# jankammeth/BA-path-planning

Hardware: AMD Instinct MI355X
Metric: SCP iterations/sec (N agents x K waypoints) (higher is better)
Workload: dtype f64

## Files before the change

### ba-path-planning_amd/csrc/scp_qp_persist16.hip

```cpp
#include "scp_qp_persist_device.h"

namespace {
using namespace scpdev;
using namespace scp_persist;

#ifdef SCP_PHASE_PROFILE
__device__ unsigned long long scp_persist16_clk[16];
#define PSTAMP(slot)                                           \
  do {                                                         \
    if (prof_t) {                                              \
      const unsigned long long now_ = wall_clock64();          \
      pacc_s[slot] += now_ - pacc_s[15];                       \
      pacc_s[15] = now_;                                       \
    }                                                          \
  } while (0)
#else
#define PSTAMP(slot) ((void)0)
#endif

constexpr int nct_of(int D, int APB) { return (D * APB + 15) / 16; }
constexpr int AB_STRIDE = 32;

constexpr bool t_on_mfma(int D, int APB) { return 4 * nct_of(D, APB) < APB && APB <= 8; }
constexpr int ent_doubles(int D) { return D + 6; }

struct Lds16 {
  int RSK, tK, nks;
  size_t rt, pt, qt, ml, tl, gp, ab, gchk, ent, n_dbl;
  __host__ __device__ Lds16(int K, int cap, int nblk, int D, int APB) {
    const int NC16 = 16 * nct_of(D, APB), APB16 = APB;
    const bool tq = t_on_mfma(D, APB);
    RSK = pad_col(K);
    tK = (K + 15) >> 4;
    nks = (K + 3) >> 2;
    size_t o = 0;
    rt = o; o += (size_t)NC16 * RSK;
    pt = o; o += (size_t)NC16 * RSK;
    ml = o; o += (size_t)tK * nks * 64;
    qt = pt;
    tl = ml;
    if (tq) {
      qt = o; o += (size_t)NC16 * RSK;
      tl = o; o += (size_t)tK * nks * 64;
    }
    gp = o; o += (size_t)2 * nblk;
    ab = o; o += (size_t)APB16 * AB_STRIDE;
    if ((size_t)2 * NC16 * RSK >= (size_t)NCHK * nblk) gchk = rt;
    else { gchk = o; o += (size_t)NCHK * nblk; }
    ent = o; o += (size_t)cap * ent_doubles(D);
    n_dbl = o;
  }
};

template <int D, int APB16>
__global__ __launch_bounds__(64 * APB16) void cg1_persist16_kernel(PersistArgs A) {
  constexpr int NT16 = 64 * APB16;
  constexpr int NCT = nct_of(D, APB16);
  constexpr int NC16 = 16 * NCT;
  constexpr bool TQ = t_on_mfma(D, APB16);
  extern __shared__ __attribute__((aligned(16))) double lds[];
  __shared__ double red[NCHK][APB16];
  __shared__ double cert_s[3][APB16];
  __shared__ double chk_s[NCHK];
  __shared__ int fail_s;
#ifdef SCP_PHASE_PROFILE
  __shared__ unsigned long long pacc_s[16];
  const bool prof_t = blockIdx.x == gridDim.x / 2 && threadIdx.x == 0;
  if (prof_t) {
    for (int i = 0; i < 15; ++i) pacc_s[i] = 0;
    pacc_s[15] = wall_clock64();
  }
#endif
  const int K = A.K, N = A.N;
  const int64_t C = A.C;
  const int cap = A.ent_cap, nblk = A.nblk;
  const Lds16 L(K, cap, nblk, D, APB16);
  const int RSK = L.RSK, tK = L.tK, nks = L.nks;
  double* Rt = lds + L.rt;
  double* Pt = lds + L.pt;
  double* Qt = lds + L.qt;
  double* Ml = lds + L.ml;
  double* Tl = lds + L.tl;
  double* gp = lds + L.gp;
  double* ab = lds + L.ab;
  double* gck = lds + L.gchk;
  double* e_c = lds + L.ent;
  double* e_l = e_c + (size_t)cap * D;
  double* e_z = e_l + cap;
  double* e_y = e_z + cap;
  double* e_g = e_y + cap;
  double* e_ax = e_g + cap;
  double* e_s = e_ax + cap;
  int* e_code = (int*)(lds + L.n_dbl);
  int* cptr = e_code + cap;

  const int wave = threadIdx.x >> 6, lane = threadIdx.x & 63;
  const int a0 = blockIdx.x * APB16;
  const int agent = a0 + wave;
  const bool aok = agent < N;
  const int k = lane;
  const bool live = aok && k < K;
  const bool jok = live && k < K - 1;
  const bool lastk = k == K - 1;
  const double h = A.h, hh = h * h, ih = 1.0 / h, alpha = A.alpha;
  double rho = A.rho, rho_c = A.rho_c;
  unsigned n_rho = 0;

  const int a1 = min(a0 + APB16, N);
  const int ebase = A.cell_ptr[cell_of(0, a0, K)];
  const int ne = A.cell_ptr[cell_of(0, a1, K)] - ebase;
  if (entries_overflow<APB16>(A)) return;
  if (threadIdx.x == 0) fail_s = 0;
  for (int i = threadIdx.x; i <= (a1 - a0) * K; i += NT16) cptr[i] = A.cell_ptr[cell_of(0, a0, K) + i] - ebase;
  for (int e = threadIdx.x; e < ne; e += NT16) {
    const int code = A.ent_code[ebase + e];
    const int n = code >> 1, side = code & 1;
    const int wi = A.w_i[n], wj = A.w_j[n], wk = A.w_k[n];
    const int own = side ? wj : wi, par = side ? wi : wj;
    e_code[e] = wk | ((own - a0) << 6) | (side << 10) | (par << 11);
    const int64_t bo = (int64_t)wk * C + (int64_t)own * D, bp = (int64_t)wk * C + (int64_t)par * D;
    double ax = 0.0;
#pragma unroll
    for (int d = 0; d < D; ++d) {
      const double eta = A.w_eta[(size_t)n * D + d];
      const double c = side ? -eta : eta;
      e_c[(size_t)e * D + d] = c;
      ax += c * (A.Qx[bo + d] - A.Qx[bp + d]);
    }
    e_ax[e] = ax;
    e_l[e] = A.w_l[n];
    e_z[e] = A.zc[n];
    e_y[e] = A.yc[n];
    e_g[e] = A.gval[ebase + e];
  }
  for (int i = threadIdx.x; i < NC16 * RSK; i += NT16) Rt[i] = 0.0;
  for (int i = threadIdx.x; i < tK * nks * 64; i += NT16) {
    Ml[i] = A.pMinv[i];
    if constexpr (TQ) Tl[i] = A.pT[i];
  }

  double v[D][4], off[D], x[D], c1[D], c2[D];
#pragma unroll
  for (int t = 0; t < 4; ++t) {
    const bool rok = t == 0 ? jok : live;
    const int row = t == 0 ? k : t * K - 1 + k;
    const double rr = (t >= 2 && lastk) ? rho * A.rho_eq : rho;
#pragma unroll
    for (int d = 0; d < D; ++d) {
      v[d][t] = 0.0;
      if (rok) {
        const int64_t g = (int64_t)row * C + (int64_t)agent * D + d;
        v[d][t] = A.zf[g] + A.yf[g] / rr;
      }
    }
  }
  if (threadIdx.x < APB16 * D) {
    const int al = threadIdx.x / D, d = threadIdx.x % D, ag = a0 + al;
    double* o = ab + al * AB_STRIDE;
    const bool there = ag < N;
    const double v0 = there ? A.states[((size_t)N + ag) * D + d] : 0.0;
    o[d] = A.vel_lo - v0;
    o[4 + d] = A.vel_hi - v0;
    o[8 + d] = (there ? A.states[((size_t)3 * N + ag) * D + d] : 0.0) - v0;
    o[12 + d] = A.pmin[d];
    o[16 + d] = A.pmax[d];
    o[20 + d] = there ? A.states[((size_t)2 * N + ag) * D + d] : 0.0;
    o[24 + d] = -1e300;
    o[28 + d] = 1e300;
  }
#pragma unroll
  for (int d = 0; d < D; ++d) {
#pragma clang fp contract(off)
    const double p0 = aok ? A.states[(size_t)agent * D + d] : 0.0, v0 = aok ? A.states[((size_t)N + agent) * D + d] : 0.0;
    const double hk = h * (double)(k + 1);
    const double hkv = hk * v0;
    off[d] = p0 + hkv;
  }
  const double* const tb = ab + wave * AB_STRIDE;
  const double* const b_vl = tb + (live ? (lastk ? 8 : 0) : 24);
  const double* const b_vh = tb + (live ? (lastk ? 8 : 4) : 28);
  const double* const b_pl = tb + (live ? (lastk ? 20 : 12) : 24);
  const double* const b_ph = tb + (live ? (lastk ? 20 : 16) : 28);
  auto bounds = [&](int d, double (&lo)[2], double (&hi)[2]) {
    lo[0] = b_vl[d];
    hi[0] = b_vh[d];
    lo[1] = b_pl[d] - off[d];
    hi[1] = b_ph[d] - off[d];
  };
#pragma unroll
  for (int d = 0; d < D; ++d) {
    x[d] = live ? A.x[(int64_t)k * C + (int64_t)agent * D + d] : 0.0;
    const double s1 = wave_incl_sum(x[d]);
    const double s2 = lane_below(wave_incl_sum(s1));
    c1[d] = live ? s1 : 0.0;
    c2[d] = live ? s2 : 0.0;
  }
  const double jlo = A.jerk_lo, jhi = A.jerk_hi, alo = A.acc_lo, ahi = A.acc_hi;
  __syncthreads();
  const int c0 = aok ? cptr[wave * K + min(k, K - 1)] : 0;
  const int c1e = (aok && k < K) ? cptr[wave * K + k + 1] : c0;
  const bool has_rows = c1e > c0;
  u64* my_cell = A.cells + ((size_t)((int64_t)min(k, K - 1) * N + (aok ? agent : 0)) * D) * 2;
  double* my_pt = Pt + (size_t)(wave * D) * RSK + k;
  double* my_rt = Rt + (size_t)(wave * D) * RSK + k;

  PSTAMP(0);
  bool ok = true;
  int it_done = A.it0;
  unsigned steps = 0;
  unsigned exit_code = 0;
  const bool with_dy = A.eps_prim_inf > 0.0;
  if (threadIdx.x < 3 * APB16) (&cert_s[0][0])[threadIdx.x] = 0.0;
  int cad = A.cad0;
  for (;;) {
  int nit = cad - it_done % cad;
  if (it_done + nit > A.max_iter) nit = A.max_iter - it_done;
  for (int it = 0; it < nit; ++it, ++steps) {
    const unsigned tag = A.epoch0 + steps + 1u;
    const bool last = it == nit - 1;
    const bool first = A.first_step && steps == 0u;
    u64* gpart = A.gpart + (size_t)(tag & 1u) * nblk * 4;
    const double rv = lastk ? rho * A.rho_eq : rho;
    {
      double r[D];
      double g[D];
#pragma unroll
      for (int d = 0; d < D; ++d) g[d] = 0.0;
      for (int e = c0; e < c1e; ++e) {
        const double ge = e_g[e];
#pragma unroll
        for (int d = 0; d < D; ++d) g[d] += e_c[(size_t)e * D + d] * ge;
      }
#pragma unroll
      for (int d = 0; d < D; ++d) {
        double lo[2], hi[2];
        bounds(d, lo, hi);
        const double xn = lane_above(x[d]);
        double cj = fmin(fmax(v[d][0], jlo), jhi), ca = fmin(fmax(v[d][1], alo), ahi);
        double cv = fmin(fmax(v[d][2], lo[0]), hi[0]), cp = fmin(fmax(v[d][3], lo[1]), hi[1]);
        if (first) { cj = v[d][0]; ca = v[d][1]; cv = v[d][2]; cp = v[d][3]; }
        const double wj = jok ? rho * ((cj - (xn - x[d]) * ih) - (v[d][0] - cj)) : 0.0;
        const double wa = rho * ((ca - x[d]) - (v[d][1] - ca));
        const double wv = rv * ((cv - h * c1[d]) - (v[d][2] - cv));
        const double wp = rv * ((cp - hh * (c2[d] + 0.5 * c1[d])) - (v[d][3] - cp));
        const double u1 = h * wv + 0.5 * hh * (wp - g[d]);
        const double u2 = wp + g[d];
        const double d1 = wave_incl_rsum(u1);
        const double s1 = wave_incl_rsum(u2);
        const double d2 = lane_above(wave_incl_rsum(s1));
        const double wjm = lane_below(wj);
        r[d] = (((wjm - wj) * ih + wa) + (d1 + 0.5 * hh * g[d]) + hh * d2) - 2.0 * x[d];
        if (live) my_rt[d * RSK] = r[d];
        __builtin_amdgcn_sched_barrier(0);
      }
    }
    __syncthreads();
    PSTAMP(1);
    if ((wave < 4 * NCT || (TQ && wave < 4 * NCT + 4)) && (wave & 3) < tK) {
      const bool tw = TQ && wave >= 4 * NCT;
      const int li = lane & 15, lk = lane >> 4;
      const int tile = wave & 3, ct = tw ? 0 : wave >> 2;
      const double* Mt = (tw ? Tl : Ml) + (size_t)tile * nks * 64 + lane;
      const double* Bt = Rt + (size_t)(ct * 16 + li) * RSK;
      double4_t acc = {0.0, 0.0, 0.0, 0.0};
#pragma unroll 4
      for (int s = 0; s < nks; ++s) {
        const int kk = 4 * s + lk;
        const double b = kk < K ? Bt[kk] : 0.0;
        acc = __builtin_amdgcn_mfma_f64_16x16x4f64(Mt[(size_t)s * 64], b, acc, 0, 0, 0);
      }
      if (TQ && tw) {
        const int al = li / D, d = li % D;
        const bool col_ok = li < D * APB16 && a0 + al < N;
        double* Ot = Qt + (size_t)li * RSK;
#pragma unroll
        for (int q = 0; q < 4; ++q) {
          const int row = tile * 16 + lk + 4 * q;
          if (row < K) {
            Ot[row] = acc[q];
            if (col_ok && cptr[al * K + row + 1] > cptr[al * K + row])
              st_granules(A.cells + ((size_t)((int64_t)row * N + a0 + al) * D + d) * 2, tag, acc[q]);
          }
        }
      } else {
        double* Ot = Pt + (size_t)(ct * 16 + li) * RSK;
#pragma unroll
        for (int q = 0; q < 4; ++q) {
          const int row = tile * 16 + lk + 4 * q;
          if (row < K) Ot[row] = acc[q];
        }
      }
    }
    __syncthreads();
    PSTAMP(2);
    double p[D], s1p[D], s2p[D];
    {
      double rz = 0.0;
#pragma unroll
      for (int d = 0; d < D; ++d) {
        p[d] = live ? my_pt[d * RSK] : 0.0;
        rz += (live ? my_rt[d * RSK] : 0.0) * p[d];
        const double cs1 = wave_incl_sum(p[d]);
        const double cs2 = lane_below(wave_incl_sum(cs1));
        s1p[d] = live ? cs1 : 0.0;
        s2p[d] = live ? cs2 : 0.0;
        if constexpr (!TQ) {
          const double qp = hh * (cs2 - 0.5 * lane_below(cs1));
          if (has_rows) {
            st_granules(my_cell + 2 * d, tag, qp);
            my_pt[d * RSK] = qp;
          }
        }
      }
      rz = wave_incl_sum(rz);
      if (lane == 63) red[0][wave] = rz;
    }
    if constexpr (!TQ) __syncthreads();
    PSTAMP(3);
    {
      double sq = 0.0;
      unsigned spins = 0;
      bool bad = false;
      for (int e = threadIdx.x; e < ne; e += NT16) {
        const int code = e_code[e];
        const int ek = code & 63, al = (code >> 6) & 15, side = (code >> 10) & 1, par = code >> 11;
        const u64* pc = A.cells + ((size_t)((int64_t)ek * N + par) * D) * 2;
        u32x4 w[D];
        if (!wait_cell<D>(A, pc, tag, spins, w)) {
          bad = true;
          break;
        }
        double s = 0.0;
#pragma unroll
        for (int d = 0; d < D; ++d) s += e_c[(size_t)e * D + d] * (Qt[(size_t)(al * D + d) * RSK + ek] - pair_value(w[d]));
        e_s[e] = s;
        if (!side) sq += s * s;
      }
      if (bad) raise_give_up(A, fail_s);
      sq = wave_incl_sum(sq);
      if (lane == 63) red[1][wave] = sq;
    }
    __syncthreads();
    if (fail_s) { ok = false; break; }
    PSTAMP(4);
    publish_partials(red, 2, 3u, gpart + (size_t)blockIdx.x * 4, tag);
    double zcl[D][4];
#pragma unroll
    for (int d = 0; d < D; ++d) {
      double lo[2], hi[2];
      bounds(d, lo, hi);
      zcl[d][0] = fmin(fmax(v[d][0], jlo), jhi);
      zcl[d][1] = fmin(fmax(v[d][1], alo), ahi);
      zcl[d][2] = fmin(fmax(v[d][2], lo[0]), hi[0]);
      zcl[d][3] = fmin(fmax(v[d][3], lo[1]), hi[1]);
      if (first) {
#pragma unroll
        for (int t = 0; t < 4; ++t) zcl[d][t] = v[d][t];
      }
    }
    gather_pairs<NT16>(A, gpart, 2 * nblk, tag, gp, fail_s);
    __syncthreads();
    if (fail_s) { ok = false; break; }
    PSTAMP(5);
    const double a = step_length(gp, nblk, rho_c);
    const double aa = alpha * a;
    PSTAMP(6);
    {
      const double irc = 1.0 / rho_c;
      for (int e = threadIdx.x; e < ne; e += NT16) {
        const double s = e_s[e], ax0 = e_ax[e];
        const double tc = fma(a, s, ax0), ax = fma(aa, s, ax0);
        e_ax[e] = ax;
        const double zo = e_z[e], yo = e_y[e];
        const double zh = alpha * tc + (1.0 - alpha) * zo;
        const double zn = fmax(zh + yo * irc, e_l[e]);
        const double yn = yo + rho_c * (zh - zn);
        e_z[e] = zn;
        e_y[e] = yn;
        e_g[e] = (rho_c * zn - yn) - rho_c * ax;
        if (last && with_dy) e_s[e] = fmin(yn - yo, 0.0);
      }
    }
    const bool cert = last && with_dy;
    if (cert) __syncthreads();
    double m_ndy = 0.0, m_supp = 0.0, m_natdy = 0.0;
    {
#pragma unroll
      for (int d = 0; d < D; ++d) {
        const double xt = fma(a, p[d], x[d]);
        const double t1 = fma(a, s1p[d], c1[d]), t2 = fma(a, s2p[d], c2[d]);
        const double xtn = lane_above(xt);
        const double cj = zcl[d][0], ca = zcl[d][1], cv = zcl[d][2], cp = zcl[d][3];
        const double nj = jok ? fma(alpha, (xtn - xt) * ih - cj, v[d][0]) : v[d][0];
        const double na = fma(alpha, xt - ca, v[d][1]);
        const double nv = fma(alpha, h * t1 - cv, v[d][2]);
        const double np = fma(alpha, hh * (t2 + 0.5 * t1) - cp, v[d][3]);
        if (cert) {
          double lo[2], hi[2];
          bounds(d, lo, hi);
          const double dyj = rho * ((nj - fmin(fmax(nj, jlo), jhi)) - (v[d][0] - cj));
          const double dya = rho * ((na - fmin(fmax(na, alo), ahi)) - (v[d][1] - ca));
          const double dyv = rv * ((nv - fmin(fmax(nv, lo[0]), hi[0])) - (v[d][2] - cv));
          const double dyp = rv * ((np - fmin(fmax(np, lo[1]), hi[1])) - (v[d][3] - cp));
          m_ndy = fmax(m_ndy, fmax(fmax(fabs(dyj), fabs(dya)), fmax(fabs(dyv), fabs(dyp))));
          m_supp += (jhi * fmax(dyj, 0.0) + jlo * fmin(dyj, 0.0)) + (ahi * fmax(dya, 0.0) + alo * fmin(dya, 0.0)) +
                    (hi[0] * fmax(dyv, 0.0) + lo[0] * fmin(dyv, 0.0)) + (hi[1] * fmax(dyp, 0.0) + lo[1] * fmin(dyp, 0.0));
          double gd = 0.0;
          for (int e = c0; e < c1e; ++e) gd += e_c[(size_t)e * D + d] * e_s[e];
          const double u1 = h * dyv + 0.5 * hh * (dyp - gd);
          const double u2 = dyp + gd;
          const double d1 = wave_incl_rsum(u1);
          const double s1 = wave_incl_rsum(u2);
          const double d2 = lane_above(wave_incl_rsum(s1));
          const double vjm = lane_below(dyj);
          const double at = ((vjm - dyj) * ih + dya) + (d1 + 0.5 * hh * gd) + hh * d2;
          if (live) m_natdy = fmax(m_natdy, fabs(at));
        }
        v[d][0] = nj; v[d][1] = na; v[d][2] = nv; v[d][3] = np;
        x[d] = fma(aa, p[d], x[d]);
        c1[d] = fma(aa, s1p[d], c1[d]);
        c2[d] = fma(aa, s2p[d], c2[d]);
        __builtin_amdgcn_sched_barrier(0);
      }
    }
    if (cert) {
      m_ndy = wave_max_nn(m_ndy);
      m_supp = wave_incl_sum(m_supp);
      m_natdy = wave_max_nn(m_natdy);
      if (lane == 63) { cert_s[0][wave] = m_ndy; cert_s[1][wave] = m_supp; cert_s[2][wave] = m_natdy; }
    }
    __syncthreads();
    PSTAMP(7);
  }

  if (!ok) break;
  it_done += nit;
  {
    const unsigned ctag = 0x80000000u | (A.epoch0 + steps);
    const double rv = lastk ? rho * A.rho_eq : rho;
    double m[NCHK];
#pragma unroll
    for (int j = 0; j < NCHK; ++j) m[j] = 0.0;
    {
      double gy[D];
#pragma unroll
      for (int d = 0; d < D; ++d) gy[d] = 0.0;
      for (int e = c0; e < c1e; ++e) {
        const double ye = e_y[e];
#pragma unroll
        for (int d = 0; d < D; ++d) gy[d] += e_c[(size_t)e * D + d] * ye;
      }
#pragma unroll
      for (int d = 0; d < D; ++d) {
        const double s1 = wave_incl_sum(x[d]);
        const double s2 = lane_below(wave_incl_sum(s1));
        const double qx = hh * (s2 - 0.5 * lane_below(s1));
        c1[d] = live ? s1 : 0.0;
        c2[d] = live ? s2 : 0.0;
        if (has_rows) {
          st_granules(my_cell + 2 * d, ctag, qx);
          my_pt[d * RSK] = qx;
        }
        double lo[2], hi[2];
        bounds(d, lo, hi);
        const double xn = lane_above(x[d]);
        const double f[4] = {jok ? (xn - x[d]) * ih : 0.0, x[d], h * c1[d], hh * (c2[d] + 0.5 * c1[d])};
        const double zc[4] = {fmin(fmax(v[d][0], jlo), jhi), fmin(fmax(v[d][1], alo), ahi),
                              fmin(fmax(v[d][2], lo[0]), hi[0]), fmin(fmax(v[d][3], lo[1]), hi[1])};
#pragma unroll
        for (int t = 0; t < 4; ++t) {
          if (t == 0 ? jok : live) {
            m[CK_RP] = fmax(m[CK_RP], fabs(f[t] - zc[t]));
            m[CK_NAX] = fmax(m[CK_NAX], fabs(f[t]));
            m[CK_NZ] = fmax(m[CK_NZ], fabs(zc[t]));
          }
        }
        const double vj = jok ? rho * (v[d][0] - zc[0]) : 0.0, va = rho * (v[d][1] - zc[1]);
        const double vv = rv * (v[d][2] - zc[2]), vp = rv * (v[d][3] - zc[3]);
        const double g = gy[d];
        const double u1 = h * vv + 0.5 * hh * (vp - g);
        const double u2 = vp + g;
        const double d1 = wave_incl_rsum(u1);
        const double r1 = wave_incl_rsum(u2);
        const double d2 = lane_above(wave_incl_rsum(r1));
        const double vjm = lane_below(vj);
        const double at = ((vjm - vj) * ih + va) + (d1 + 0.5 * hh * g) + hh * d2;
        if (live) {
          const double px = 2.0 * x[d];
          m[CK_RD] = fmax(m[CK_RD], fabs(px + at));
          m[CK_NPX] = fmax(m[CK_NPX], fabs(px));
          m[CK_NATY] = fmax(m[CK_NATY], fabs(at));
        }
        __builtin_amdgcn_sched_barrier(0);
      }
    }
    __syncthreads();
    {
      unsigned spins = 0;
      bool bad = false;
      for (int e = threadIdx.x; e < ne; e += NT16) {
        const int code = e_code[e];
        const int ek = code & 63, al = (code >> 6) & 15, side = (code >> 10) & 1, par = code >> 11;
        const u64* pc = A.cells + ((size_t)((int64_t)ek * N + par) * D) * 2;
        u32x4 w[D];
        if (!wait_cell<D>(A, pc, ctag, spins, w)) {
          bad = true;
          break;
        }
        double ax = 0.0;
#pragma unroll
        for (int d = 0; d < D; ++d) {
          const double qq = pair_value(w[d]);
          const double qo = Pt[(size_t)(al * D + d) * RSK + ek];
          ax += e_c[(size_t)e * D + d] * (qo - qq);
        }
        e_ax[e] = ax;
        if (!side) {
          const double zc_ = e_z[e];
          m[CK_RP] = fmax(m[CK_RP], fabs(ax - zc_));
          m[CK_NAX] = fmax(m[CK_NAX], fabs(ax));
          m[CK_NZ] = fmax(m[CK_NZ], fabs(zc_));
          if (with_dy) {
            const double dd = e_s[e];
            m[CK_NDY] = fmax(m[CK_NDY], fabs(dd));
            m[CK_SUPP] += e_l[e] * dd;
          }
        }
      }
      if (bad) raise_give_up(A, fail_s);
    }
#pragma unroll
    for (int j = 0; j < NCHK; ++j) {
      double v = j == CK_SUPP ? wave_incl_sum(m[j]) : wave_max_nn(m[j]);
      if (lane == 63) {
        if (j == CK_NDY) v = fmax(v, cert_s[0][wave]);
        if (j == CK_SUPP) v += cert_s[1][wave];
        if (j == CK_NATDY) v = fmax(v, cert_s[2][wave]);
        red[j][wave] = v;
      }
    }
    __syncthreads();
    if (fail_s) { ok = false; break; }
    publish_partials(red, NCHK, 1u << CK_SUPP, A.gcheck + (size_t)blockIdx.x * NCHK * 2, ctag);
    gather_pairs<NT16>(A, A.gcheck, NCHK * nblk, ctag, gck, fail_s);
    __syncthreads();
    if (fail_s) { ok = false; break; }
    double chk[NCHK];
    reduce_checks(gck, nblk, chk);
    if (threadIdx.x == 0) {
#pragma unroll
      for (int j = 0; j < NCHK; ++j) chk_s[j] = chk[j];
    }
    __syncthreads();
    if (L.gchk == L.rt) {
      for (int i = threadIdx.x; i < NC16 * RSK; i += NT16) Rt[i] = 0.0;
    }
    int slot;
    exit_code = check_decision(A, chk, it_done, rho, with_dy, cad, slot);
    if (exit_code) break;
    if (slot >= 0) {
      const double nrs = A.tab[slot].rho;
      {
#pragma unroll
        for (int d = 0; d < D; ++d) {
          double lo[2], hi[2];
          bounds(d, lo, hi);
          const double zc[4] = {fmin(fmax(v[d][0], jlo), jhi), fmin(fmax(v[d][1], alo), ahi),
                                fmin(fmax(v[d][2], lo[0]), hi[0]), fmin(fmax(v[d][3], lo[1]), hi[1])};
#pragma unroll
          for (int t = 0; t < 4; ++t) {
            const double rr_old = (t >= 2 && lastk) ? rho * A.rho_eq : rho, rr_new = (t >= 2 && lastk) ? nrs * A.rho_eq : nrs;
            const double yv = rr_old * (v[d][t] - zc[t]);
            v[d][t] = zc[t] + yv / rr_new;
          }
        }
      }
      rho = nrs;
      rho_c = rho * A.rho_col_scale;
      for (int i = threadIdx.x; i < tK * nks * 64; i += NT16) {
        Ml[i] = A.tab[slot].pMinv[i];
        if constexpr (TQ) Tl[i] = A.tab[slot].pT[i];
      }
      for (int e = threadIdx.x; e < ne; e += NT16)
        e_g[e] = (rho_c * e_z[e] - e_y[e]) - rho_c * e_ax[e];
      ++n_rho;
    }
    __syncthreads();
    PSTAMP(9);
  }
  }

  if (leave_if_gave_up(A, ok)) return;
#pragma unroll
  for (int d = 0; d < D; ++d) {
    const double xn = lane_above(x[d]);
    const double c1b = lane_below(c1[d]);
    double lo[2], hi[2];
    bounds(d, lo, hi);
    const double f[4] = {(xn - x[d]) * ih, x[d], h * c1[d], hh * (c2[d] + 0.5 * c1[d])};
    const double zc[4] = {fmin(fmax(v[d][0], jlo), jhi), fmin(fmax(v[d][1], alo), ahi),
                          fmin(fmax(v[d][2], lo[0]), hi[0]), fmin(fmax(v[d][3], lo[1]), hi[1])};
#pragma unroll
    for (int t = 0; t < 4; ++t) {
      if (t == 0 ? jok : live) {
        const int row = t == 0 ? k : t * K - 1 + k;
        const int64_t g = (int64_t)row * C + (int64_t)agent * D + d;
        A.zf[g] = zc[t];
        A.yf[g] = ((t >= 2 && lastk) ? rho * A.rho_eq : rho) * (v[d][t] - zc[t]);
        A.fx[g] = f[t];
      }
    }
    if (live) {
      const int64_t g = (int64_t)k * C + (int64_t)agent * D + d;
      A.x[g] = x[d];
      A.Qx[g] = hh * (c2[d] - 0.5 * c1b);
    }
  }
  for (int e = threadIdx.x; e < ne; e += NT16) {
    A.gval[ebase + e] = e_g[e];
    if (!((e_code[e] >> 10) & 1)) {
      const int n = A.ent_code[ebase + e] >> 1;
      A.zc[n] = e_z[e];
      A.yc[n] = e_y[e];
    }
  }
  PSTAMP(8);
#ifdef SCP_PHASE_PROFILE
  if (prof_t)
    for (int i = 0; i < 16; ++i) scp_persist16_clk[i] = i == 15 ? (unsigned long long)steps : pacc_s[i];
#endif
  publish_exit(A, chk_s, it_done, n_rho, rho, exit_code);
}

}

#ifdef SCP_PHASE_PROFILE
extern "C" int scp_debug_persist16_clocks(unsigned long long* out, int n) {
  if (n > 16) n = 16;
  return hipMemcpyFromSymbol(out, HIP_SYMBOL(scp_persist16_clk), (size_t)n * sizeof(unsigned long long)) == hipSuccess ? 0 : 1;
}
#endif

size_t scp_persist16_entry_bytes(int D) { return (size_t)ent_doubles(D) * sizeof(double) + sizeof(int); }

size_t scp_persist16_lds_bytes(int K, int cap, int nblk, int D, int apb) {
  const Lds16 L(K, cap, nblk, D, apb);
  const size_t ints = (size_t)cap + (size_t)apb * K + 1;
  return L.n_dbl * sizeof(double) + ((ints + 1) / 2 * 2) * sizeof(int);
}

KernelFn scp_persist16_kernel(int D, int apb) {
  if (D == 2 && apb == 16) return cg1_persist16_kernel<2, 16>;
  if (D == 2 && apb == 8) return cg1_persist16_kernel<2, 8>;
  if (D == 3 && apb == 8) return cg1_persist16_kernel<3, 8>;
  return nullptr;
}
```

### ba-path-planning_amd/csrc/scp_qp_persist_device.h

```cpp
#pragma once
#include "scp_qp_device.h"

#if defined(__HIP_DEVICE_COMPILE__) && !defined(__gfx950__)
#error "scp_qp_persist_device.h: the persistent ADMM kernels' hand-offs are written for gfx950 only"
#endif

namespace scp_persist {
using namespace scpdev;

typedef unsigned long long u64;
constexpr unsigned SPIN_LIMIT = 1u << 20;

struct PersistArgs {
  int K, N, nblk, ent_cap;
  int it0, max_iter, check_every, rho_interval;
  int cad0, check_fine;
  double fine_ratio;
  int64_t C;
  double rho, rho_c, rho_eq, alpha, h;
  double eps_abs, eps_rel, eps_prim_inf, rho_tol;
  double jerk_lo, jerk_hi, acc_lo, acc_hi, vel_lo, vel_hi, pmin[3], pmax[3];
  const double* states;
  int first_step;
  int spin_sleep;
  const double* pMinv;
  const double* pT;
  const double *lf, *uf;
  double *zf, *yf, *fx, *x, *Qx, *dyf;
  u64* cells;
  u64* gpart;
  u64* gcheck;
  unsigned* give_up;
  const int *cell_ptr, *ent_code, *w_k, *w_i, *w_j;
  const double *w_eta, *w_l;
  double *zc, *yc, *dyc, *gval;
  unsigned* host_status;
  double* host_scal;
  u64* host_flag;
  u64 seq;
  unsigned epoch0;
  double rho_col_scale;
  double* host_rho;
  int n_tab;
  struct RhoSlot {
    double rho;
    const double* pMinv;
    const double* pT;
  } tab[SCP_KKT_SLOTS_MAX];
};

typedef void (*KernelFn)(PersistArgs);

enum { EXIT_SOLVED = 1, EXIT_GAVE_UP = 2, EXIT_MAX_ITER = 3, EXIT_INFEASIBLE = 4, EXIT_RHO = 5, EXIT_OVERFLOW = 6 };
constexpr int NCHK = 9;
constexpr int CK_RP = 0, CK_NAX = 1, CK_NZ = 2, CK_RD = 3, CK_NPX = 4, CK_NATY = 5, CK_NDY = 6, CK_SUPP = 7, CK_NATDY = 8;

typedef unsigned int u32x4 __attribute__((ext_vector_type(4)));
__device__ inline void st_granules(u64* g, unsigned tag, double v) {
  const u32x4 w = {(unsigned)__double2loint(v), tag, (unsigned)__double2hiint(v), tag};
  asm volatile("global_store_dwordx4 %0, %1, off sc1\n\ts_nop 1" ::"v"(g), "v"(w) : "memory");
}
__device__ inline u32x4 ld_pair(const u64* g) {
  u32x4 w;
  asm volatile("global_load_dwordx4 %0, %1, off sc1\n\ts_waitcnt vmcnt(0)" : "=v"(w) : "v"(g) : "memory");
  return w;
}
template <int D>
__device__ inline void ld_cell(const u64* g, u32x4 (&w)[D]) {
  if (D == 2) {
    asm volatile("global_load_dwordx4 %0, %2, off sc1\n\tglobal_load_dwordx4 %1, %2, off offset:16 sc1\n\ts_waitcnt vmcnt(0)"
                 : "=&v"(w[0]), "=&v"(w[1])
                 : "v"(g)
                 : "memory");
  } else {
#pragma unroll
    for (int d = 0; d < D; ++d) w[d] = ld_pair(g + 2 * d);
  }
}
__device__ inline void spin_nap(int n) {
  for (int i = 0; i < n; ++i) __builtin_amdgcn_s_sleep(1);
}
__device__ inline bool pair_ok(const u32x4& w, unsigned tag) { return w[1] == tag && w[3] == tag; }
__device__ inline double pair_value(const u32x4& w) { return __hiloint2double((int)w[2], (int)w[0]); }


template <int D>
__device__ __forceinline__ bool wait_cell(const PersistArgs& A, const u64* g, unsigned tag, unsigned& spins, u32x4 (&w)[D]) {
  for (;;) {
    ld_cell<D>(g, w);
    bool here = true;
#pragma unroll
    for (int d = 0; d < D; ++d) here = here && pair_ok(w[d], tag);
    if (here) return true;
    if (++spins > SPIN_LIMIT ||
        ((spins & 255u) == 0u && __hip_atomic_load(A.give_up, __ATOMIC_RELAXED, __HIP_MEMORY_SCOPE_AGENT) != 0u))
      return false;
    spin_nap(A.spin_sleep);
  }
}

__device__ __forceinline__ void raise_give_up(const PersistArgs& A, int& fail_s) {
  __hip_atomic_store(A.give_up, 1u, __ATOMIC_RELAXED, __HIP_MEMORY_SCOPE_AGENT);
  fail_s = 1;
}

template <int APB>
__device__ __forceinline__ void publish_partials(const double (&red)[NCHK][APB], int n, unsigned sum_mask, u64* dst,
                                                 unsigned tag) {
  if (threadIdx.x < n) {
    const int j = threadIdx.x;
    double t = 0.0;
#pragma unroll
    for (int w = 0; w < APB; ++w) t = (sum_mask >> j) & 1u ? t + red[j][w] : fmax(t, red[j][w]);
    st_granules(dst + 2 * j, tag, t);
  }
}

template <int NT>
__device__ __forceinline__ void gather_pairs(const PersistArgs& A, const u64* buf, int n, unsigned tag, double* out,
                                             int& fail_s) {
  unsigned spins = 0;
  bool bad = false;
  for (int q = threadIdx.x; q < n; q += NT) {
    u32x4 w[1];
    if (!wait_cell<1>(A, buf + 2 * q, tag, spins, w)) {
      bad = true;
      break;
    }
    out[q] = pair_value(w[0]);
  }
  if (bad) raise_give_up(A, fail_s);
}

__device__ __forceinline__ double step_length(const double* gp, int nblk, double rho_c) {
  double vr = 0.0, vs = 0.0;
  for (int b = threadIdx.x & 63; b < nblk; b += 64) {
    vr += gp[2 * b];
    vs += gp[2 * b + 1];
  }
  const double rzt = read_lane(wave_incl_sum(vr), 63);
  const double sqt = read_lane(wave_incl_sum(vs), 63);
  const double pHp = rzt + rho_c * sqt;
  return (pHp > 0.0 && rzt != 0.0) ? rzt / pHp : 0.0;
}

__device__ __forceinline__ void reduce_checks(const double* gck, int nblk, double (&chk)[NCHK]) {
#pragma unroll
  for (int j = 0; j < NCHK; ++j) {
    double v = 0.0;
    for (int b = threadIdx.x & 63; b < nblk; b += 64) v = j == CK_SUPP ? v + gck[b * NCHK + j] : fmax(v, gck[b * NCHK + j]);
    chk[j] = read_lane(j == CK_SUPP ? wave_incl_sum(v) : wave_max_nn(v), 63);
  }
}

__device__ __forceinline__ unsigned check_decision(const PersistArgs& A, const double (&chk)[NCHK], int it_done, double rho,
                                                   bool with_dy, int& cad, int& slot) {
  slot = -1;
  const double np_ = fmax(chk[CK_NAX], chk[CK_NZ]), nd_ = fmax(chk[CK_NPX], chk[CK_NATY]);
  const double tol_p = A.eps_abs + A.eps_rel * np_, tol_d = A.eps_abs + A.eps_rel * nd_;
  if (chk[CK_RP] <= tol_p && chk[CK_RD] <= tol_d) return EXIT_SOLVED;
  if (A.check_fine > 0)
    cad = (chk[CK_RP] < A.fine_ratio * tol_p && chk[CK_RD] < A.fine_ratio * tol_d) ? A.check_fine : A.check_every;
  if (it_done >= A.max_iter) return EXIT_MAX_ITER;
  if (with_dy && chk[CK_NDY] > A.eps_prim_inf && chk[CK_SUPP] < -A.eps_prim_inf * chk[CK_NDY] &&
      chk[CK_NATDY] < A.eps_prim_inf * chk[CK_NDY])
    return EXIT_INFEASIBLE;
  if (A.rho_tol > 0.0 && it_done % A.rho_interval == 0) {
    const double prim = chk[CK_RP] / fmax(np_, 1e-10), dual = chk[CK_RD] / fmax(nd_, 1e-10);
    const double nr = fmin(fmax(rho * sqrt(prim / fmax(dual, 1e-10)), 1e-6), 1e6);
    const double cand = exp2(round(4.0 * log2(nr)) * 0.25);
    if (cand > rho * A.rho_tol * (1.0 - 1e-9) || cand < rho / A.rho_tol * (1.0 + 1e-9)) {
      int s = -1;
      for (int i = 0; i < A.n_tab; ++i)
        if (fabs(A.tab[i].rho - cand) <= 1e-12 * cand) s = i;
      if (s < 0) return EXIT_RHO;
      const double nrs = A.tab[s].rho;
      if (nrs > rho * A.rho_tol || nrs < rho / A.rho_tol) {
        slot = s;
        if (A.check_fine > 0) cad = A.check_fine;
      }
    }
  }
  return 0;
}

template <int APB>
__device__ __forceinline__ bool entries_overflow(const PersistArgs& A) {
  int worst = 0;
  for (int b = threadIdx.x; b < (A.N + APB - 1) / APB; b += 64 * APB) {
    const int b0 = b * APB, b1 = min(b0 + APB, A.N);
    worst = max(worst, A.cell_ptr[cell_of(0, b1, A.K)] - A.cell_ptr[cell_of(0, b0, A.K)]);
  }
  if (!__syncthreads_or(worst > A.ent_cap)) return false;
  if (blockIdx.x == 0 && threadIdx.x == 0) {
    __hip_atomic_store(A.host_status, (unsigned)EXIT_OVERFLOW, __ATOMIC_RELAXED, __HIP_MEMORY_SCOPE_SYSTEM);
    __hip_atomic_store(A.host_flag, A.seq, __ATOMIC_RELEASE, __HIP_MEMORY_SCOPE_SYSTEM);
  }
  return true;
}

__device__ __forceinline__ bool leave_if_gave_up(const PersistArgs& A, bool ok) {
  if (ok && __syncthreads_or(threadIdx.x == 0 &&
                             __hip_atomic_load(A.give_up, __ATOMIC_RELAXED, __HIP_MEMORY_SCOPE_AGENT) != 0u))
    ok = false;
  if (ok) return false;
  if (threadIdx.x == 0) {
    __hip_atomic_store(A.host_status, (unsigned)EXIT_GAVE_UP, __ATOMIC_RELAXED, __HIP_MEMORY_SCOPE_SYSTEM);
    __hip_atomic_store(A.host_flag, A.seq, __ATOMIC_RELEASE, __HIP_MEMORY_SCOPE_SYSTEM);
  }
  return true;
}

__device__ __forceinline__ void publish_exit(const PersistArgs& A, const double* chk, int it_done, unsigned n_rho, double rho,
                                             unsigned exit_code) {
  if (blockIdx.x == 0 && threadIdx.x == 0) {
    const int slot[NCHK] = {SL_RP, SL_NAX, SL_NZ, SL_RD, SL_NPX, SL_NATY, SL_NDY, SL_SUPP, SL_NATDY};
#pragma unroll
    for (int j = 0; j < NCHK; ++j)
      __hip_atomic_store((u64*)(A.host_scal + slot[j]), (u64)__double_as_longlong(chk[j]), __ATOMIC_RELAXED,
                         __HIP_MEMORY_SCOPE_SYSTEM);
    __hip_atomic_store(A.host_status + 1, (unsigned)it_done, __ATOMIC_RELAXED, __HIP_MEMORY_SCOPE_SYSTEM);
    __hip_atomic_store(A.host_status + 2, n_rho, __ATOMIC_RELAXED, __HIP_MEMORY_SCOPE_SYSTEM);
    __hip_atomic_store((u64*)A.host_rho, (u64)__double_as_longlong(rho), __ATOMIC_RELAXED, __HIP_MEMORY_SCOPE_SYSTEM);
    __hip_atomic_store(A.host_status, exit_code, __ATOMIC_RELAXED, __HIP_MEMORY_SCOPE_SYSTEM);
    __hip_atomic_store(A.host_flag, A.seq, __ATOMIC_RELEASE, __HIP_MEMORY_SCOPE_SYSTEM);
  }
}

}

size_t scp_persist16_lds_bytes(int K, int cap, int nblk, int D, int apb);
size_t scp_persist16_entry_bytes(int D);
scp_persist::KernelFn scp_persist16_kernel(int D, int apb);
```

Before: 417.2.

## Speculatively form next ADMM residual during convergence-check gather and stage final outputs via LDS

```diff
diff --git a/ba-path-planning_amd/csrc/scp_qp_persist16.hip b/ba-path-planning_amd/csrc/scp_qp_persist16.hip
--- a/ba-path-planning_amd/csrc/scp_qp_persist16.hip
+++ b/ba-path-planning_amd/csrc/scp_qp_persist16.hip
@@ -6,6 +6,7 @@
 
 #ifdef SCP_PHASE_PROFILE
 __device__ unsigned long long scp_persist16_clk[16];
+__device__ unsigned long long scp_persist16_tot[4];
 #define PSTAMP(slot)                                           \
   do {                                                         \
     if (prof_t) {                                              \
@@ -27,26 +28,28 @@
 struct Lds16 {
   int RSK, tK, nks;
   size_t rt, pt, qt, ml, tl, gp, ab, gchk, ent, n_dbl;
+  bool spec;
   __host__ __device__ Lds16(int K, int cap, int nblk, int D, int APB) {
     const int NC16 = 16 * nct_of(D, APB), APB16 = APB;
     const bool tq = t_on_mfma(D, APB);
     RSK = pad_col(K);
     tK = (K + 15) >> 4;
     nks = (K + 3) >> 2;
+    const size_t tile = (size_t)NC16 * RSK, need = (size_t)NCHK * nblk;
     size_t o = 0;
-    rt = o; o += (size_t)NC16 * RSK;
-    pt = o; o += (size_t)NC16 * RSK;
+    rt = o; o += tile;
+    pt = o; o += tile;
+    qt = pt;
+    if (tq) { qt = o; o += tile; }
     ml = o; o += (size_t)tK * nks * 64;
-    qt = pt;
     tl = ml;
-    if (tq) {
-      qt = o; o += (size_t)NC16 * RSK;
-      tl = o; o += (size_t)tK * nks * 64;
-    }
+    if (tq) { tl = o; o += (size_t)tK * nks * 64; }
     gp = o; o += (size_t)2 * nblk;
     ab = o; o += (size_t)APB16 * AB_STRIDE;
-    if ((size_t)2 * NC16 * RSK >= (size_t)NCHK * nblk) gchk = rt;
-    else { gchk = o; o += (size_t)NCHK * nblk; }
+    spec = true;
+    if (2 * tile < need) { gchk = o; o += need; }
+    else if ((tq ? 2 : 1) * tile >= need) gchk = pt;
+    else { gchk = rt; spec = false; }
     ent = o; o += (size_t)cap * ent_doubles(D);
     n_dbl = o;
   }
@@ -211,6 +214,41 @@
   unsigned exit_code = 0;
   const bool with_dy = A.eps_prim_inf > 0.0;
   if (threadIdx.x < 3 * APB16) (&cert_s[0][0])[threadIdx.x] = 0.0;
+  auto form_r = [&](const bool first) __attribute__((always_inline)) {
+    const double rv = lastk ? rho * A.rho_eq : rho;
+    double r[D];
+    double g[D];
+#pragma unroll
+    for (int d = 0; d < D; ++d) g[d] = 0.0;
+    for (int e = c0; e < c1e; ++e) {
+      const double ge = e_g[e];
+#pragma unroll
+      for (int d = 0; d < D; ++d) g[d] += e_c[(size_t)e * D + d] * ge;
+    }
+#pragma unroll
+    for (int d = 0; d < D; ++d) {
+      double lo[2], hi[2];
+      bounds(d, lo, hi);
+      const double xn = lane_above(x[d]);
+      double cj = fmin(fmax(v[d][0], jlo), jhi), ca = fmin(fmax(v[d][1], alo), ahi);
+      double cv = fmin(fmax(v[d][2], lo[0]), hi[0]), cp = fmin(fmax(v[d][3], lo[1]), hi[1]);
+      if (first) { cj = v[d][0]; ca = v[d][1]; cv = v[d][2]; cp = v[d][3]; }
+      const double wj = jok ? rho * ((cj - (xn - x[d]) * ih) - (v[d][0] - cj)) : 0.0;
+      const double wa = rho * ((ca - x[d]) - (v[d][1] - ca));
+      const double wv = rv * ((cv - h * c1[d]) - (v[d][2] - cv));
+      const double wp = rv * ((cp - hh * (c2[d] + 0.5 * c1[d])) - (v[d][3] - cp));
+      const double u1 = h * wv + 0.5 * hh * (wp - g[d]);
+      const double u2 = wp + g[d];
+      const double d1 = wave_incl_rsum(u1);
+      const double s1 = wave_incl_rsum(u2);
+      const double d2 = lane_above(wave_incl_rsum(s1));
+      const double wjm = lane_below(wj);
+      r[d] = (((wjm - wj) * ih + wa) + (d1 + 0.5 * hh * g[d]) + hh * d2) - 2.0 * x[d];
+      if (live) my_rt[d * RSK] = r[d];
+      __builtin_amdgcn_sched_barrier(0);
+    }
+  };
+  bool r_formed = false;
   int cad = A.cad0;
   for (;;) {
   int nit = cad - it_done % cad;
@@ -221,40 +259,15 @@
     const bool first = A.first_step && steps == 0u;
     u64* gpart = A.gpart + (size_t)(tag & 1u) * nblk * 4;
     const double rv = lastk ? rho * A.rho_eq : rho;
-    {
-      double r[D];
-      double g[D];
-#pragma unroll
-      for (int d = 0; d < D; ++d) g[d] = 0.0;
-      for (int e = c0; e < c1e; ++e) {
-        const double ge = e_g[e];
-#pragma unroll
-        for (int d = 0; d < D; ++d) g[d] += e_c[(size_t)e * D + d] * ge;
-      }
-#pragma unroll
-      for (int d = 0; d < D; ++d) {
-        double lo[2], hi[2];
-        bounds(d, lo, hi);
-        const double xn = lane_above(x[d]);
-        double cj = fmin(fmax(v[d][0], jlo), jhi), ca = fmin(fmax(v[d][1], alo), ahi);
-        double cv = fmin(fmax(v[d][2], lo[0]), hi[0]), cp = fmin(fmax(v[d][3], lo[1]), hi[1]);
-        if (first) { cj = v[d][0]; ca = v[d][1]; cv = v[d][2]; cp = v[d][3]; }
-        const double wj = jok ? rho * ((cj - (xn - x[d]) * ih) - (v[d][0] - cj)) : 0.0;
-        const double wa = rho * ((ca - x[d]) - (v[d][1] - ca));
-        const double wv = rv * ((cv - h * c1[d]) - (v[d][2] - cv));
-        const double wp = rv * ((cp - hh * (c2[d] + 0.5 * c1[d])) - (v[d][3] - cp));
-        const double u1 = h * wv + 0.5 * hh * (wp - g[d]);
-        const double u2 = wp + g[d];
-        const double d1 = wave_incl_rsum(u1);
-        const double s1 = wave_incl_rsum(u2);
-        const double d2 = lane_above(wave_incl_rsum(s1));
-        const double wjm = lane_below(wj);
-        r[d] = (((wjm - wj) * ih + wa) + (d1 + 0.5 * hh * g[d]) + hh * d2) - 2.0 * x[d];
-        if (live) my_rt[d * RSK] = r[d];
-        __builtin_amdgcn_sched_barrier(0);
-      }
-    }
-    __syncthreads();
+    if (r_formed) {
+      r_formed = false;
+#ifdef SCP_PHASE_PROFILE
+      if (prof_t) ++pacc_s[14];
+#endif
+    } else {
+      form_r(first);
+      __syncthreads();
+    }
     PSTAMP(1);
     if ((wave < 4 * NCT || (TQ && wave < 4 * NCT + 4)) && (wave & 3) < tK) {
       const bool tw = TQ && wave >= 4 * NCT;
@@ -437,10 +450,25 @@
   it_done += nit;
   {
     const unsigned ctag = 0x80000000u | (A.epoch0 + steps);
+#ifdef SCP_PHASE_PROFILE
+    if (prof_t) ++pacc_s[13];
+#endif
     const double rv = lastk ? rho * A.rho_eq : rho;
     double m[NCHK];
 #pragma unroll
     for (int j = 0; j < NCHK; ++j) m[j] = 0.0;
+#pragma unroll
+    for (int d = 0; d < D; ++d) {
+      const double s1 = wave_incl_sum(x[d]);
+      const double s2 = lane_below(wave_incl_sum(s1));
+      const double qx = hh * (s2 - 0.5 * lane_below(s1));
+      c1[d] = live ? s1 : 0.0;
+      c2[d] = live ? s2 : 0.0;
+      if (has_rows) {
+        st_granules(my_cell + 2 * d, ctag, qx);
+        my_pt[d * RSK] = qx;
+      }
+    }
     {
       double gy[D];
 #pragma unroll
@@ -452,15 +480,6 @@
       }
 #pragma unroll
       for (int d = 0; d < D; ++d) {
-        const double s1 = wave_incl_sum(x[d]);
-        const double s2 = lane_below(wave_incl_sum(s1));
-        const double qx = hh * (s2 - 0.5 * lane_below(s1));
-        c1[d] = live ? s1 : 0.0;
-        c2[d] = live ? s2 : 0.0;
-        if (has_rows) {
-          st_granules(my_cell + 2 * d, ctag, qx);
-          my_pt[d * RSK] = qx;
-        }
         double lo[2], hi[2];
         bounds(d, lo, hi);
         const double xn = lane_above(x[d]);
@@ -495,6 +514,7 @@
       }
     }
     __syncthreads();
+    PSTAMP(9);
     {
       unsigned spins = 0;
       bool bad = false;
@@ -502,6 +522,13 @@
         const int code = e_code[e];
         const int ek = code & 63, al = (code >> 6) & 15, side = (code >> 10) & 1, par = code >> 11;
         const u64* pc = A.cells + ((size_t)((int64_t)ek * N + par) * D) * 2;
+        double cc[D], qo[D];
+#pragma unroll
+        for (int d = 0; d < D; ++d) {
+          cc[d] = e_c[(size_t)e * D + d];
+          qo[d] = Pt[(size_t)(al * D + d) * RSK + ek];
+        }
+        const double zc_ = e_z[e], dd_ = (with_dy && !side) ? e_s[e] : 0.0, le_ = e_l[e];
         u32x4 w[D];
         if (!wait_cell<D>(A, pc, ctag, spins, w)) {
           bad = true;
@@ -511,19 +538,16 @@
 #pragma unroll
         for (int d = 0; d < D; ++d) {
           const double qq = pair_value(w[d]);
-          const double qo = Pt[(size_t)(al * D + d) * RSK + ek];
-          ax += e_c[(size_t)e * D + d] * (qo - qq);
+          ax += cc[d] * (qo[d] - qq);
         }
         e_ax[e] = ax;
         if (!side) {
-          const double zc_ = e_z[e];
           m[CK_RP] = fmax(m[CK_RP], fabs(ax - zc_));
           m[CK_NAX] = fmax(m[CK_NAX], fabs(ax));
           m[CK_NZ] = fmax(m[CK_NZ], fabs(zc_));
           if (with_dy) {
-            const double dd = e_s[e];
-            m[CK_NDY] = fmax(m[CK_NDY], fabs(dd));
-            m[CK_SUPP] += e_l[e] * dd;
+            m[CK_NDY] = fmax(m[CK_NDY], fabs(dd_));
+            m[CK_SUPP] += le_ * dd_;
           }
         }
       }
@@ -541,7 +565,10 @@
     }
     __syncthreads();
     if (fail_s) { ok = false; break; }
+    PSTAMP(10);
     publish_partials(red, NCHK, 1u << CK_SUPP, A.gcheck + (size_t)blockIdx.x * NCHK * 2, ctag);
+    const bool r_ahead = L.spec && steps > 0u;
+    if (r_ahead) form_r(false);
     gather_pairs<NT16>(A, A.gcheck, NCHK * nblk, ctag, gck, fail_s);
     __syncthreads();
     if (fail_s) { ok = false; break; }
@@ -551,8 +578,9 @@
 #pragma unroll
       for (int j = 0; j < NCHK; ++j) chk_s[j] = chk[j];
     }
-    __syncthreads();
+    PSTAMP(11);
     if (L.gchk == L.rt) {
+      __syncthreads();
       for (int i = threadIdx.x; i < NC16 * RSK; i += NT16) Rt[i] = 0.0;
     }
     int slot;
@@ -585,35 +613,67 @@
         e_g[e] = (rho_c * e_z[e] - e_y[e]) - rho_c * e_ax[e];
       ++n_rho;
     }
+    r_formed = r_ahead && slot < 0;
     __syncthreads();
-    PSTAMP(9);
+    PSTAMP(12);
   }
   }
 
   if (leave_if_gave_up(A, ok)) return;
-#pragma unroll
-  for (int d = 0; d < D; ++d) {
-    const double xn = lane_above(x[d]);
-    const double c1b = lane_below(c1[d]);
-    double lo[2], hi[2];
-    bounds(d, lo, hi);
-    const double f[4] = {(xn - x[d]) * ih, x[d], h * c1[d], hh * (c2[d] + 0.5 * c1[d])};
-    const double zc[4] = {fmin(fmax(v[d][0], jlo), jhi), fmin(fmax(v[d][1], alo), ahi),
-                          fmin(fmax(v[d][2], lo[0]), hi[0]), fmin(fmax(v[d][3], lo[1]), hi[1])};
-#pragma unroll
-    for (int t = 0; t < 4; ++t) {
-      if (t == 0 ? jok : live) {
-        const int row = t == 0 ? k : t * K - 1 + k;
-        const int64_t g = (int64_t)row * C + (int64_t)agent * D + d;
-        A.zf[g] = zc[t];
-        A.yf[g] = ((t >= 2 && lastk) ? rho * A.rho_eq : rho) * (v[d][t] - zc[t]);
-        A.fx[g] = f[t];
-      }
-    }
-    if (live) {
-      const int64_t g = (int64_t)k * C + (int64_t)agent * D + d;
-      A.x[g] = x[d];
-      A.Qx[g] = hh * (c2[d] - 0.5 * c1b);
+  {
+    constexpr int NCW = APB16 * D, NSL = TQ ? 3 : 2, NITEM = 14;
+    const size_t tile = (size_t)NC16 * RSK;
+    const int rs = (size_t)(NCW + 1) * K <= tile ? NCW + 1 : NCW;
+    const int ncol = (a1 - a0) * D;
+    double* const arr[3] = {A.zf, A.yf, A.fx};
+#pragma unroll
+    for (int j0 = 0; j0 < NITEM; j0 += NSL) {
+      if (j0) __syncthreads();
+#pragma unroll
+      for (int s = 0; s < NSL; ++s) {
+        const int j = j0 + s;
+        if (j < NITEM) {
+          double* const slab = Rt + s * tile + (size_t)k * rs + wave * D;
+#pragma unroll
+          for (int d = 0; d < D; ++d) {
+            double val;
+            bool on = live;
+            if (j < 12) {
+              const int t = j / 3, a = j % 3;
+              on = t == 0 ? jok : live;
+              double lo[2], hi[2];
+              bounds(d, lo, hi);
+              const double zc = t == 0 ? fmin(fmax(v[d][0], jlo), jhi) : t == 1 ? fmin(fmax(v[d][1], alo), ahi)
+                              : t == 2 ? fmin(fmax(v[d][2], lo[0]), hi[0]) : fmin(fmax(v[d][3], lo[1]), hi[1]);
+              if (a == 0) val = zc;
+              else if (a == 1) val = ((t >= 2 && lastk) ? rho * A.rho_eq : rho) * (v[d][t] - zc);
+              else val = t == 0 ? (lane_above(x[d]) - x[d]) * ih : t == 1 ? x[d] : t == 2 ? h * c1[d] : hh * (c2[d] + 0.5 * c1[d]);
+            } else if (j == 12) {
+              val = x[d];
+            } else {
+              const double c1b = lane_below(c1[d]);
+              val = hh * (c2[d] - 0.5 * c1b);
+            }
+            if (on) slab[d] = val;
+          }
+        }
+      }
+      __syncthreads();
+#pragma unroll
+      for (int s = 0; s < NSL; ++s) {
+        const int j = j0 + s;
+        if (j < NITEM) {
+          const int t = j / 3;
+          const int nr = j < 3 ? K - 1 : K;
+          const int row0 = (j < 12 && t > 0) ? t * K - 1 : 0;
+          double* const dst = (j < 12 ? arr[j % 3] : j == 12 ? A.x : A.Qx) + (int64_t)row0 * C + (int64_t)a0 * D;
+          const double* const src = Rt + s * tile;
+          for (int i = threadIdx.x; i < nr * NCW; i += NT16) {
+            const int row = i / NCW, c = i - row * NCW;
+            if (c < ncol) dst[(int64_t)row * C + c] = src[row * rs + c];
+          }
+        }
+      }
     }
   }
   for (int e = threadIdx.x; e < ne; e += NT16) {
@@ -626,8 +686,13 @@
   }
   PSTAMP(8);
 #ifdef SCP_PHASE_PROFILE
-  if (prof_t)
+  if (prof_t) {
     for (int i = 0; i < 16; ++i) scp_persist16_clk[i] = i == 15 ? (unsigned long long)steps : pacc_s[i];
+    scp_persist16_tot[0] += 1;
+    scp_persist16_tot[1] += steps;
+    scp_persist16_tot[2] += pacc_s[13];
+    scp_persist16_tot[3] += pacc_s[14];
+  }
 #endif
   publish_exit(A, chk_s, it_done, n_rho, rho, exit_code);
 }
@@ -639,6 +704,10 @@
   if (n > 16) n = 16;
   return hipMemcpyFromSymbol(out, HIP_SYMBOL(scp_persist16_clk), (size_t)n * sizeof(unsigned long long)) == hipSuccess ? 0 : 1;
 }
+extern "C" int scp_debug_persist16_totals(unsigned long long* out, int n) {
+  if (n > 4) n = 4;
+  return hipMemcpyFromSymbol(out, HIP_SYMBOL(scp_persist16_tot), (size_t)n * sizeof(unsigned long long)) == hipSuccess ? 0 : 1;
+}
 #endif
 
 size_t scp_persist16_entry_bytes(int D) { return (size_t)ent_doubles(D) * sizeof(double) + sizeof(int); }
@@ -647,6 +716,11 @@
   const Lds16 L(K, cap, nblk, D, apb);
   const size_t ints = (size_t)cap + (size_t)apb * K + 1;
   return L.n_dbl * sizeof(double) + ((ints + 1) / 2 * 2) * sizeof(int);
+}
+
+int scp_persist16_gather_place(int K, int nblk, int D, int apb) {
+  const Lds16 L(K, 0, nblk, D, apb);
+  return L.gchk == L.pt ? 0 : L.spec ? 1 : 2;
 }
 
 KernelFn scp_persist16_kernel(int D, int apb) {
diff --git a/ba-path-planning_amd/csrc/scp_qp_persist_device.h b/ba-path-planning_amd/csrc/scp_qp_persist_device.h
--- a/ba-path-planning_amd/csrc/scp_qp_persist_device.h
+++ b/ba-path-planning_amd/csrc/scp_qp_persist_device.h
@@ -231,4 +231,5 @@
 
 size_t scp_persist16_lds_bytes(int K, int cap, int nblk, int D, int apb);
 size_t scp_persist16_entry_bytes(int D);
+int scp_persist16_gather_place(int K, int nblk, int D, int apb);
 scp_persist::KernelFn scp_persist16_kernel(int D, int apb);
```

Result: slower. 398.8 (-4.4%).
